# laizesheng1/Monte-Carlo-Path-Tracer

Measured on AMD Instinct MI355X. Metric: Mray/s (primary+secondary), cornell-box 1024spp, higher is better.
Workload: dtype f32; 1 GPU; S-cornell (synthetic cornell-box.obj stand-in, 39612 tris) 800x800, depth=8, 1024 spp per step, MIS integrator, reference-faithful shadow rays; spp_per_rank=1024, n_tris=39612, wide_bvh=8-wide, 4220 nodes, depth 9, scene_device_bytes=21940128, parallelism=sample-range shard x1 + RCCL all-reduce of the 800x800x4 fp32 film

## Files before the change

### monte-carlo-path-tracer_amd/csrc/device_scene.h

```cpp
#pragma once
#include <stdint.h>
#include <hip/hip_runtime.h>

#ifndef MCPT_Q_MARGIN
#define MCPT_Q_MARGIN (1.0 / 1024.0)
#endif
#ifndef MCPT_LEAF_MAX
#define MCPT_LEAF_MAX 2
#endif
#ifndef MCPT_STACK_DEPTH
#define MCPT_STACK_DEPTH 64
#endif
#ifndef MCPT_BLOCK
#define MCPT_BLOCK 256
#endif
#ifndef MCPT_TOP_NODES
#define MCPT_TOP_NODES 256
#endif
#define MCPT_NODE_SENTINEL ((int)0x80000000)
#define HIT_CLASS_SHIFT 28
#define HIT_TRI_MASK 0x0fffffff
#define HIT_CLASS_DIFFUSE 0u
#define HIT_CLASS_PHONG 1u
#define HIT_CLASS_MIRROR 2u
// ... 29 lines not shown
#define MCPT_N8_WORD(slot) ((slot) >> 1)
#define MCPT_N8_LO_SHIFT(slot) (8 * ((slot) & 1))
#define MCPT_N8_HI_SHIFT(slot) (16 + 8 * ((slot) & 1))
#define MCPT_N8_EMPTY_WORD 0x0000ffffu
#define MCPT_TRI_SHADE_F4 8
struct DevScene {
    const float4* nodes;
    const float4* nodes8;
    const float4* tri_isect;
    const float4* tri_shade;
    const double* tri_pos64;
    const int32_t* tri_face;
    const DevMaterial* mats;
    const DevLight* lights;
    const double* light_pos64;
    const float4* texels;
    DevCamera cam;
    double centre[3];
    int32_t n_tris, n_lights, n_nodes, n_mats, n_nodes8;
};

struct RenderParams {
    uint32_t spp;
    uint32_t first_sample;
    uint32_t samples_per_item;
    uint32_t chunks;
    uint32_t tiles_x, tiles_y;
    uint32_t tile_mod, tile_rem;
    uint32_t n_owned;
    uint32_t max_depth;
    uint32_t flags;
    uint32_t integrator;
    uint32_t seed_lo, seed_hi;
    uint32_t atomic_accum;
// ... 16 lines not shown
```

### monte-carlo-path-tracer_amd/csrc/mcpt_api.cpp

```cpp
#include "../../include/mcpt.h"
#include "kernels.h"
#include "scene_build.h"
#include "bvh_gpu.h"
#include "wavefront.h"
#include "denoise.h"
#include "adaptive.h"
#include "refit.h"

#include <chrono>
#include <cmath>
#include <cstdlib>
#include <cstdio>
#include <cstring>
#include <memory>
#include <string>
#include <vector>

namespace {

thread_local std::string g_err;

template <class H, auto Free> struct Owned {
    H h = nullptr;
    Owned() = default;
// ... 16 lines not shown
    void release() { if (p) { (void)hipFree(p); if (tally) *tally -= bytes; } p = nullptr; bytes = 0; }
    hipError_t alloc(size_t n, uint64_t* count = nullptr) {
        release();
        const hipError_t e = hipMalloc(&p, n ? n : 16);
        if (e == hipSuccess) { bytes = n; tally = count; if (tally) *tally += n; } else p = nullptr;
        return e;
    }
};

}

struct mcpt_ctx {
    int device = 0;
    mcpt_opts opts{};
    DevScene dev{};
    DevBuf nodes, nodes8, tri_isect, tri_shade, tri_pos64, tri_face, mats, lights, light_pos64, texels, accum_own, counters;
    float4* accum = nullptr;
    Stream own_stream; hipStream_t stream = nullptr;
    static constexpr uint32_t TIMED = 16;
    Event ev0[TIMED], ev1[TIMED];
    uint32_t timed_head = 0, timed_tail = 0;
    double last_kernel_ms = 0.0, total_kernel_ms = 0.0;
    uint64_t launches = 0;
    mcpt_scene_info info{};
    int width = 0, height = 0;
    bool use_wavefront = true;
    struct WfLane {
        PathPool pool{};
        CompactBufs compact{};
        std::vector<DevBuf> pool_bufs;
        DevBuf ctl_buf, ovf_buf;
// ... 169 lines not shown
                HIP_TRY(hipStreamCreateWithFlags(L.stream.out(), hipStreamNonBlocking));
                const size_t ovf_bytes = size_t(c->trace_grid) * wf_trace_block_threads() * wf_trace_overflow_bytes_per_lane(c->wide_depth);
                if (ovf_bytes > (size_t(512) << 20)) return fail(MCPT_ERR_BVH_DEPTH, "wide BVH of depth " + std::to_string(c->wide_depth) + " needs a traversal-stack overflow area of " + std::to_string(ovf_bytes >> 20) + " MB per sub-pipeline: build the tree with the host builder (no MCPT_FLAG_GPU_BVH_BUILD)");
                HIP_TRY(L.ovf_buf.alloc(ovf_bytes));
            }
        }
    }
    HIP_TRY(hipDeviceSynchronize());
    c->accum = static_cast<float4*>(c->accum_own.p);
    DevScene& d = c->dev;
    d.nodes = static_cast<const float4*>(c->nodes.p); d.nodes8 = static_cast<const float4*>(c->nodes8.p);
    d.tri_isect = static_cast<const float4*>(c->tri_isect.p);
    d.tri_shade = static_cast<const float4*>(c->tri_shade.p); d.tri_pos64 = static_cast<const double*>(c->tri_pos64.p);
    d.tri_face = static_cast<const int32_t*>(c->tri_face.p); d.mats = static_cast<const DevMaterial*>(c->mats.p);
    d.lights = static_cast<const DevLight*>(c->lights.p); d.light_pos64 = static_cast<const double*>(c->light_pos64.p); d.texels = static_cast<const float4*>(c->texels.p);
    return MCPT_OK;
}

static void fill_wide_info(mcpt_scene_info& in, const HostScene& hs) {
    in.wide_width = 8; in.wide_nodes = uint32_t(hs.nodes8.size() / 5);
    in.wide_depth = hs.bvh8_depth;
    in.traversal_bytes = (hs.nodes8.size() + hs.tri_isect.size()) * sizeof(f4h);
    for (int a = 0; a < 3; a++) in.centre[a] = hs.centre[a];
    uint64_t h = 1469598103934665603ull;
    auto mix = [&](const void* p, size_t bytes) { const uint32_t* w = static_cast<const uint32_t*>(p); for (size_t i = 0; i < bytes / 4; i++) { h ^= w[i]; h *= 1099511628211ull; } };
    mix(hs.nodes8.data(), hs.nodes8.size() * sizeof(f4h)); mix(hs.tri_face.data(), hs.tri_face.size() * 4);
    in.wide_tree_hash = h;
}


// ... 100 lines not shown
        if ((st = check_device(o.device)) != MCPT_OK) return st;
    }

    if ((hs.nodes8.size() * sizeof(f4h) >= (1ull << 32) || hs.tri_isect.size() * sizeof(f4h) >= (1ull << 32)))
        return fail(MCPT_ERR_UNSUPPORTED, "scene too large for the 8-wide traversal kernel (more than 89 M triangles)");
    std::unique_ptr<mcpt_ctx, void (*)(mcpt_ctx*)> guard(new mcpt_ctx(), destroy_ctx);
    mcpt_ctx* c = guard.get();
    c->device = o.device; c->opts = o; c->width = scene->camera.width; c->height = scene->camera.height;
    c->wide_depth = hs.bvh8_depth; c->binary_ok = hs.binary_ok; c->use_wavefront = use_wavefront;
    HIP_TRY(hipSetDevice(c->device));
    auto t0 = std::chrono::steady_clock::now();
    uint64_t* tally = &c->info.device_bytes;
    HIP_TRY(upload(c->nodes, hs.nodes, tally)); HIP_TRY(upload(c->nodes8, hs.nodes8, tally)); HIP_TRY(upload(c->tri_isect, hs.tri_isect, tally));
    HIP_TRY(upload(c->tri_shade, hs.tri_shade, tally)); HIP_TRY(upload(c->tri_pos64, hs.tri_pos64, tally)); HIP_TRY(upload(c->tri_face, hs.tri_face, tally));
    HIP_TRY(upload(c->mats, hs.mats, tally)); HIP_TRY(upload(c->lights, hs.lights, tally)); HIP_TRY(upload(c->light_pos64, hs.light_pos64, tally));
    HIP_TRY(upload(c->texels, hs.texels, tally));
    DevScene& d = c->dev;
    d.n_nodes8 = int32_t(hs.nodes8.size() / 5);
    d.cam = hs.cam;
    for (int a = 0; a < 3; a++) d.centre[a] = hs.centre[a];
    d.n_tris = int32_t(hs.tri_face.size()); d.n_lights = int32_t(hs.lights.size()); d.n_nodes = int32_t(hs.nodes.size() / 4); d.n_mats = int32_t(hs.mats.size());
    mcpt_scene_info& in = c->info;
    in.n_tris = uint32_t(d.n_tris); in.n_lights = uint32_t(d.n_lights); in.n_nodes = uint32_t(d.n_nodes);
    in.bvh_depth = hs.bvh_depth; in.max_leaf = hs.max_leaf; in.width = uint32_t(c->width); in.height = uint32_t(c->height);
    in.bvh_build_ms = hs.bvh_build_ms;
    fill_wide_info(in, hs);
    if ((st = finish_ctx(c)) != MCPT_OK) return st;
    if ((o.flags & MCPT_FLAG_DYNAMIC) && (st = rf_setup(c, hs, scene)) != MCPT_OK) return st;
    in.upload_ms = std::chrono::duration<double, std::milli>(std::chrono::steady_clock::now() - t0).count();
    *out_ctx = guard.release();
    return MCPT_OK;
}

mcpt_status mcpt_clone_to_device(mcpt_ctx* src, int32_t device, mcpt_ctx** out_ctx) {
    if (!src || !out_ctx) return fail(MCPT_ERR_INVALID_ARG, "mcpt_clone_to_device: null argument");
    *out_ctx = nullptr;
    mcpt_status st = check_device(device); if (st != MCPT_OK) return st;
    st = use(src); if (st != MCPT_OK) return st;
    HIP_TRY(hipStreamSynchronize(src->stream));
    std::unique_ptr<mcpt_ctx, void (*)(mcpt_ctx*)> guard(new mcpt_ctx(), destroy_ctx);
    mcpt_ctx* c = guard.get();
    c->device = device; c->opts = src->opts; c->opts.device = device; c->width = src->width; c->height = src->height;
    c->wide_depth = src->wide_depth; c->binary_ok = src->binary_ok; c->use_wavefront = src->use_wavefront;
    c->dev = src->dev; c->info = src->info; c->info.bvh_build_ms = 0.0; c->info.device_bytes = 0;
    HIP_TRY(hipSetDevice(device));
    auto t0 = std::chrono::steady_clock::now();
    DevBuf* from[10] = {&src->nodes, &src->nodes8, &src->tri_isect, &src->tri_shade, &src->tri_pos64, &src->tri_face, &src->mats, &src->lights, &src->light_pos64, &src->texels};
    DevBuf* to[10] = {&c->nodes, &c->nodes8, &c->tri_isect, &c->tri_shade, &c->tri_pos64, &c->tri_face, &c->mats, &c->lights, &c->light_pos64, &c->texels};
    for (int i = 0; i < 10; i++) {
        HIP_TRY(to[i]->alloc(from[i]->bytes, &c->info.device_bytes));
        if (from[i]->bytes) HIP_TRY(hipMemcpyPeer(to[i]->p, device, from[i]->p, src->device, from[i]->bytes));
    }
    if ((st = finish_ctx(c)) != MCPT_OK) return st;
    if (src->dynamic && (st = rf_clone(c, src)) != MCPT_OK) return st;
    c->info.upload_ms = std::chrono::duration<double, std::milli>(std::chrono::steady_clock::now() - t0).count();
    *out_ctx = guard.release();
    return MCPT_OK;
}

mcpt_status mcpt_destroy(mcpt_ctx* ctx) {
    if (!ctx) return MCPT_OK;
    (void)hipSetDevice(ctx->device);
    (void)hipDeviceSynchronize();
    destroy_ctx(ctx);
// ... 625 lines not shown
    if (ctx->rf_timed) { HIP_TRY(hipEventSynchronize(ctx->rf_ev1)); float ms = 0.f; HIP_TRY(hipEventElapsedTime(&ms, ctx->rf_ev0, ctx->rf_ev1)); ctx->rf_last_ms = ms; ctx->rf_timed = false; }
    const size_t vd = size_t(n_vertex) * 3, nd = size_t(ctx->rf_n_normal) * 3;
    std::memcpy(ctx->rf_stage, vertex, vd * sizeof(double));
    if (normal) std::memcpy(ctx->rf_stage + vd, normal, nd * sizeof(double));
    hipStream_t s = ctx->stream;
    HIP_TRY(hipEventRecord(ctx->rf_ev0, s));
    HIP_TRY(hipMemcpyAsync(ctx->rf_vtx.p, ctx->rf_stage, vd * sizeof(double), hipMemcpyHostToDevice, s));
    if (normal) HIP_TRY(hipMemcpyAsync(ctx->rf_nrm.p, ctx->rf_stage + vd, nd * sizeof(double), hipMemcpyHostToDevice, s));
    HIP_TRY(hipEventRecord(ctx->rf_stage_ev, s)); ctx->rf_stage_pending = true;
    const double* d_nrm = normal ? static_cast<const double*>(ctx->rf_nrm.p) : nullptr;
    const int32_t* idx = static_cast<const int32_t*>(ctx->rf_idx.p);
    float* tri_box = static_cast<float*>(ctx->rf_tri_box.p);
    const DevScene& d = ctx->dev;
    HIP_TRY(launch_rf_triangles(static_cast<const double*>(ctx->rf_vtx.p), d_nrm, idx, RfCentre{d.centre[0], d.centre[1], d.centre[2]}, static_cast<float4*>(ctx->tri_isect.p),
                                static_cast<float4*>(ctx->tri_shade.p), static_cast<double*>(ctx->tri_pos64.p), tri_box, uint32_t(d.n_tris), s));
    HIP_TRY(launch_rf_lights(static_cast<DevLight*>(ctx->lights.p), static_cast<double*>(ctx->light_pos64.p), d.tri_isect, d.tri_pos64, d_nrm, idx, uint32_t(d.n_lights), s));
    for (size_t k = 0; k + 1 < ctx->rf_bin_level.size(); k++)
        HIP_TRY(launch_rf_binary_level(static_cast<float4*>(ctx->nodes.p), static_cast<const uint32_t*>(ctx->rf_bin_order.p), ctx->rf_bin_level[k], ctx->rf_bin_level[k + 1], tri_box, s));
    for (size_t k = ctx->rf_wide_level.size() - 1; k-- > 0;)
        HIP_TRY(launch_rf_wide_level(static_cast<float4*>(ctx->nodes8.p), ctx->rf_wide_level[k], ctx->rf_wide_level[k + 1], tri_box, static_cast<float*>(ctx->rf_node_box.p), s));
    HIP_TRY(launch_rf_wide_area(d.nodes8, uint32_t(d.n_nodes8), static_cast<double*>(ctx->rf_area.p), s));
    HIP_TRY(hipEventRecord(ctx->rf_ev1, s)); ctx->rf_timed = true;
    ctx->rf_updates++;
    rf_forget_derived(ctx);
    return MCPT_OK;
}

mcpt_status mcpt_get_update_info(mcpt_ctx* ctx, mcpt_update_info* out) {
    mcpt_status st = use(ctx); if (st != MCPT_OK) return st;
    if (!out) return fail(MCPT_ERR_INVALID_ARG, "null output");
    HIP_TRY(hipStreamSynchronize(ctx->stream));
// ... 231 lines not shown
```

### monte-carlo-path-tracer_amd/csrc/refit.h

```cpp
#pragma once
#include <hip/hip_runtime.h>
#include "device_scene.h"

#define RF_BLOCK 256

struct RfCentre { double x, y, z; };

hipError_t launch_rf_triangles(const double* vertex, const double* normal, const int32_t* idx6, RfCentre centre, float4* tri_isect, float4* tri_shade,
                               double* tri_pos64, float* tri_box, uint32_t n_tris, hipStream_t stream);
hipError_t launch_rf_lights(DevLight* lights, double* light_pos64, const float4* tri_isect, const double* tri_pos64, const double* normal,
                            const int32_t* idx6, uint32_t n_lights, hipStream_t stream);
hipError_t launch_rf_binary_level(float4* nodes, const uint32_t* order, uint32_t begin, uint32_t end, const float* tri_box, hipStream_t stream);
hipError_t launch_rf_wide_level(float4* nodes8, uint32_t begin, uint32_t end, const float* tri_box, float* node_box, hipStream_t stream);
hipError_t launch_rf_wide_area(const float4* nodes8, uint32_t n_nodes8, double* partial, hipStream_t stream);
inline uint32_t rf_area_blocks(uint32_t n_nodes8) { return (n_nodes8 + RF_BLOCK - 1) / RF_BLOCK; }
```

### monte-carlo-path-tracer_amd/csrc/refit.hip

```cpp
#include "refit.h"

#pragma clang fp contract(off)

namespace {

__device__ __forceinline__ float rf_down(double v) { float f = (float)v; if ((double)f > v) f = nextafterf(f, -INFINITY); return f; }
__device__ __forceinline__ float rf_up(double v) { float f = (float)v; if ((double)f < v) f = nextafterf(f, INFINITY); return f; }

struct RfBox { float lo[3], hi[3]; };
__device__ __forceinline__ RfBox rf_load_box(const float* __restrict__ boxes, size_t i) {
    const float2* p = reinterpret_cast<const float2*>(boxes + 6 * i);
    const float2 a = p[0], b = p[1], c = p[2];
    return RfBox{{a.x, a.y, b.x}, {b.y, c.x, c.y}};
}
__device__ __forceinline__ void rf_store_box(float* __restrict__ boxes, size_t i, const RfBox& b) {
    float2* p = reinterpret_cast<float2*>(boxes + 6 * i);
    p[0] = make_float2(b.lo[0], b.lo[1]); p[1] = make_float2(b.lo[2], b.hi[0]); p[2] = make_float2(b.hi[1], b.hi[2]);
}
__device__ __forceinline__ void rf_grow(RfBox& a, const RfBox& b) {
    for (int x = 0; x < 3; x++) { a.lo[x] = fminf(a.lo[x], b.lo[x]); a.hi[x] = fmaxf(a.hi[x], b.hi[x]); }
}
__device__ __forceinline__ RfBox rf_leaf_box(const float* __restrict__ tri_box, uint32_t first, uint32_t cnt) {
    RfBox b = rf_load_box(tri_box, first);
    for (uint32_t t = 1; t < cnt; t++) rf_grow(b, rf_load_box(tri_box, (size_t)first + t));
// ... 30 lines not shown
    }
    double* P = tri_pos64 + 9 * (size_t)i;
    for (int a = 0; a < 3; a++) { P[a] = v0[a]; P[3 + a] = v1[a]; P[6 + a] = v2[a]; }
    {
        const double ax = v1[0] - v0[0], ay = v1[1] - v0[1], az = v1[2] - v0[2], bx = v2[0] - v0[0], by = v2[1] - v0[1], bz = v2[2] - v0[2];
        const double nx = ay * bz - by * az, ny = az * bx - bz * ax, nz = ax * by - bx * ay;
        const double d = nx * v0[0] + ny * v0[1] + nz * v0[2];
        double2* pl = reinterpret_cast<double2*>(S + 4);
        pl[0] = make_double2(nx, ny); pl[1] = make_double2(nz, d);
    }
    RfBox b;
    for (int a = 0; a < 3; a++) { b.lo[a] = rf_down(fmin(v0[a], fmin(v1[a], v2[a]))); b.hi[a] = rf_up(fmax(v0[a], fmax(v1[a], v2[a]))); }
    rf_store_box(tri_box, i, b);
}

__global__ void __launch_bounds__(RF_BLOCK) rf_lights_kernel(DevLight* __restrict__ lights, double* __restrict__ light_pos64, const float4* __restrict__ tri_isect,
                                                             const double* __restrict__ tri_pos64, const double* __restrict__ normal, const int32_t* __restrict__ idx6,
                                                             uint32_t n_lights) {
    const uint32_t i = blockIdx.x * RF_BLOCK + threadIdx.x;
    if (i >= n_lights) return;
    float4* R = reinterpret_cast<float4*>(lights + i);
    float4 r0 = R[0], r1 = R[1], r2 = R[2], r3 = R[3];
    const uint32_t tri = (uint32_t)__float_as_int(r0.x);
    const float4 e1 = tri_isect[3 * (size_t)tri + 1], e2 = tri_isect[3 * (size_t)tri + 2];
    const float cx = e1.y * e2.z - e2.y * e1.z, cy = e1.z * e2.x - e2.z * e1.x, cz = e1.x * e2.y - e2.x * e1.y;
    r0.y = 0.5f * (float)sqrt((double)((cx * cx + cy * cy) + cz * cz));
    if (normal) {
        const int32_t* ix = idx6 + 6 * (size_t)tri + 3;
        const double* n0 = normal + 3 * (size_t)ix[0]; const double* n1 = normal + 3 * (size_t)ix[1]; const double* n2 = normal + 3 * (size_t)ix[2];
        r1.y = (float)n0[0]; r1.z = (float)n0[1]; r1.w = (float)n0[2];
        r2.x = (float)n1[0]; r2.y = (float)n1[1]; r2.z = (float)n1[2];
        r2.w = (float)n2[0]; r3.x = (float)n2[1]; r3.y = (float)n2[2];
    }
    R[0] = r0; R[1] = r1; R[2] = r2; R[3] = r3;
    for (int a = 0; a < 9; a++) light_pos64[9 * (size_t)i + a] = tri_pos64[9 * (size_t)tri + a];
}

__global__ void __launch_bounds__(RF_BLOCK) rf_binary_kernel(float4* __restrict__ nodes, const uint32_t* __restrict__ order, uint32_t begin, uint32_t end,
                                                             const float* __restrict__ tri_box) {
    const uint32_t k = begin + blockIdx.x * RF_BLOCK + threadIdx.x;
    if (k >= end) return;
    float4* N = nodes + 4 * (size_t)order[k];
    const float4 a0 = N[0], a1 = N[1], az = N[2], links = N[3];
    RfBox b[2] = {{{a0.x, a0.z, az.x}, {a0.y, a0.w, az.y}}, {{a1.x, a1.z, az.z}, {a1.y, a1.w, az.w}}};
#pragma unroll
    for (int c = 0; c < 2; c++) {
        const int code = __float_as_int(c == 0 ? links.x : links.y);
        if (code >= 0) {
            const float4* C = nodes + 4 * (size_t)code;
            const float4 c0 = C[0], c1 = C[1], cz = C[2];
// ... 99 lines not shown
    __syncthreads();
    if (threadIdx.x == 0) { double t = 0.0; for (int w = 0; w < RF_BLOCK / 64; w++) t += s_sum[w]; partial[blockIdx.x] = t; }
}

inline dim3 rf_grid(uint32_t n) { return dim3((n + RF_BLOCK - 1) / RF_BLOCK); }

}

hipError_t launch_rf_triangles(const double* vertex, const double* normal, const int32_t* idx6, RfCentre centre, float4* tri_isect, float4* tri_shade,
                               double* tri_pos64, float* tri_box, uint32_t n_tris, hipStream_t stream) {
    if (n_tris == 0) return hipSuccess;
    hipLaunchKernelGGL(rf_triangles_kernel, rf_grid(n_tris), dim3(RF_BLOCK), 0, stream, vertex, normal, idx6, centre, tri_isect, tri_shade, tri_pos64, tri_box, n_tris);
    return hipGetLastError();
}

hipError_t launch_rf_lights(DevLight* lights, double* light_pos64, const float4* tri_isect, const double* tri_pos64, const double* normal,
                            const int32_t* idx6, uint32_t n_lights, hipStream_t stream) {
    if (n_lights == 0) return hipSuccess;
    hipLaunchKernelGGL(rf_lights_kernel, rf_grid(n_lights), dim3(RF_BLOCK), 0, stream, lights, light_pos64, tri_isect, tri_pos64, normal, idx6, n_lights);
    return hipGetLastError();
}

hipError_t launch_rf_binary_level(float4* nodes, const uint32_t* order, uint32_t begin, uint32_t end, const float* tri_box, hipStream_t stream) {
    if (end <= begin) return hipSuccess;
    hipLaunchKernelGGL(rf_binary_kernel, rf_grid(end - begin), dim3(RF_BLOCK), 0, stream, nodes, order, begin, end, tri_box);
    return hipGetLastError();
}

hipError_t launch_rf_wide_level(float4* nodes8, uint32_t begin, uint32_t end, const float* tri_box, float* node_box, hipStream_t stream) {
    if (end <= begin) return hipSuccess;
    hipLaunchKernelGGL(rf_wide_kernel, rf_grid(end - begin), dim3(RF_BLOCK), 0, stream, nodes8, begin, end, tri_box, node_box);
    return hipGetLastError();
}

// ... 6 lines not shown
```

### monte-carlo-path-tracer_amd/csrc/scene_build.cpp

```cpp
#include "scene_build.h"

#include <algorithm>
#include <atomic>
#include <chrono>
#include <future>
#include <cmath>
#include <cstdio>
#include <cstdlib>
#include <cstring>
#include <limits>
#include <system_error>
#include <thread>

static constexpr double kMaxCoord = MCPT_MAX_COORD;

namespace {

struct BTri { double lo[3], hi[3], c[3]; };
struct Box {
    double lo[3], hi[3];
    Box() { for (int a = 0; a < 3; a++) { lo[a] = std::numeric_limits<double>::max(); hi[a] = std::numeric_limits<double>::lowest(); } }
    void grow(const double* l, const double* h) { for (int a = 0; a < 3; a++) { lo[a] = std::min(lo[a], l[a]); hi[a] = std::max(hi[a], h[a]); } }
    void grow(const Box& b) { grow(b.lo, b.hi); }
    void grow_pt(const double* p) { for (int a = 0; a < 3; a++) { lo[a] = std::min(lo[a], p[a]); hi[a] = std::max(hi[a], p[a]); } }
// ... 658 lines not shown
        S[1] = {float(n1[0]), float(n1[1]), float(n1[2]), float(t0_[1])};
        S[2] = {float(n2[0]), float(n2[1]), float(n2[2]), float(t1_[0])};
        S[3] = {float(t1_[1]), float(t2_[0]), float(t2_[1]), as_float(c[3])};
        for (int a = 0; a < 3; a++) { out.tri_pos64[9 * size_t(i) + a] = v0[a]; out.tri_pos64[9 * size_t(i) + 3 + a] = v1[a]; out.tri_pos64[9 * size_t(i) + 6 + a] = v2[a]; }
        {
            const double ax = v1[0] - v0[0], ay = v1[1] - v0[1], az = v1[2] - v0[2], bx = v2[0] - v0[0], by = v2[1] - v0[1], bz = v2[2] - v0[2];
            const double nx = ay * bz - by * az, ny = az * bx - bz * ax, nz = ax * by - bx * ay;
            const double pl[4] = {nx, ny, nz, nx * v0[0] + ny * v0[1] + nz * v0[2]};
            std::memcpy(&S[4], pl, sizeof pl);
        }
        out.tri_face[i] = f;
        if (out.keep_dynamic) for (int k = 0; k < 3; k++) { out.dyn_idx[6 * size_t(i) + k] = c[4 * k]; out.dyn_idx[6 * size_t(i) + 3 + k] = c[4 * k + 1]; }
    }
    });

    out.lights.clear(); out.light_pos64.clear();
    for (uint32_t f = 0; f < nf; f++) {
        const int32_t* c = d->face + 12 * size_t(f);
        const mcpt_material& m = d->materials[c[3]];
        if (!(len3(m.radiance) > 0.01)) continue;
        DevLight L; std::memset(&L, 0, sizeof L);
        L.tri = pos_of_face[f];
        const f4h e1 = out.tri_isect[3 * size_t(L.tri) + 1], e2 = out.tri_isect[3 * size_t(L.tri) + 2];
        const float cx = e1.y * e2.z - e2.y * e1.z, cy = e1.z * e2.x - e2.z * e1.x, cz = e1.x * e2.y - e2.x * e1.y;
        L.area = 0.5f * std::sqrt((cx * cx + cy * cy) + cz * cz);
        for (int a = 0; a < 3; a++) {
            L.radiance[a] = float(m.radiance[a]);
            L.n0[a] = float(d->normal[3 * size_t(c[1]) + a]); L.n1[a] = float(d->normal[3 * size_t(c[5]) + a]); L.n2[a] = float(d->normal[3 * size_t(c[9]) + a]);
        }
        out.lights.push_back(L);
        out.light_pos64.insert(out.light_pos64.end(), out.tri_pos64.begin() + 9 * size_t(L.tri), out.tri_pos64.begin() + 9 * size_t(L.tri) + 9);
    }
    if (out.lights.empty()) { err = "scene has no emissive triangle (|radiance| > 0.01); the reference indexes lights[-1] here"; return MCPT_ERR_NO_LIGHTS; }

    camera_constants(d->camera, ctr, out.cam);
    return MCPT_OK;
}
```

### monte-carlo-path-tracer_amd/csrc/scene_build.h

```cpp
#pragma once
#include <cstdint>
#include <functional>
#include <string>
#include <vector>
#include "../../include/mcpt.h"
#include "device_scene.h"

struct f4h { float x, y, z, w; };

struct HostScene {
    std::vector<f4h> nodes;
    std::vector<f4h> nodes8;
    std::vector<f4h> tri_isect;
    std::vector<f4h> tri_shade;
    std::vector<double> tri_pos64;
    std::vector<int32_t> tri_face;
    std::vector<DevMaterial> mats;
    std::vector<DevLight> lights;
    std::vector<double> light_pos64;
    std::vector<f4h> texels;
    DevCamera cam;
    double centre[3] = {0.0, 0.0, 0.0};
    uint32_t bvh_depth = 0, max_leaf = 0, bvh8_depth = 0;
    std::vector<int> subtree_begin;
    bool reference_tie_order = false;
    bool allow_deep_binary = false;
    bool binary_ok = true;
    double bvh_build_ms = 0.0;
    bool keep_dynamic = false;
    std::vector<int32_t> dyn_idx;
};

using BvhBuildFn = std::function<bool(const float* boxes, uint32_t n, std::vector<f4h>& nodes, std::vector<int>& order, uint32_t& depth,
                                      uint32_t& max_leaf, std::string& err)>;
// ... 15 lines not shown
```

### monte-carlo-path-tracer_amd/csrc/wavefront.h

```cpp
#pragma once
#include <hip/hip_runtime.h>
#include <stdint.h>
#include "device_scene.h"

#ifndef WF_SHADE_BLOCK
#define WF_SHADE_BLOCK 256
#endif
#define SLOT_DEAD  0u
#define SLOT_ALIVE 1u
#define SLOT_DRAIN 2u

struct PathPool {
    float4* ray_o;
    float4* ray_d;
    float4* hit;
    float4* sq_o;
    float4* sq_d;
    float4* nee;
    float4* L;
    float4* beta;
    float4* sum;
    uint4* ids;
    uint32_t* shadow_queue;
    uint32_t* shadow_count;
    uint32_t* live_cnt;
// ... 55 lines not shown
```

### monte-carlo-path-tracer_amd/csrc/wavefront.hip

```cpp
#include "pt_device.h"
#include "wavefront.h"

typedef float wf_v4f __attribute__((ext_vector_type(4)));
typedef unsigned int wf_v4u __attribute__((ext_vector_type(4)));
typedef double wf_v2d __attribute__((ext_vector_type(2)));
__device__ __forceinline__ float4 ld_s(const float4* p) { const wf_v4f v = __builtin_nontemporal_load(reinterpret_cast<const wf_v4f*>(p)); return make_float4(v.x, v.y, v.z, v.w); }
__device__ __forceinline__ void st_s(float4* p, float4 v) { wf_v4f t; t.x = v.x; t.y = v.y; t.z = v.z; t.w = v.w; __builtin_nontemporal_store(t, reinterpret_cast<wf_v4f*>(p)); }
__device__ __forceinline__ uint4 ld_s(const uint4* p) { const wf_v4u v = __builtin_nontemporal_load(reinterpret_cast<const wf_v4u*>(p)); return make_uint4(v.x, v.y, v.z, v.w); }
__device__ __forceinline__ void st_s(uint4* p, uint4 v) { wf_v4u t; t.x = v.x; t.y = v.y; t.z = v.z; t.w = v.w; __builtin_nontemporal_store(t, reinterpret_cast<wf_v4u*>(p)); }
__device__ __forceinline__ double4 ld_s(const double4* p) {
    const wf_v2d a = __builtin_nontemporal_load(reinterpret_cast<const wf_v2d*>(p)), b = __builtin_nontemporal_load(reinterpret_cast<const wf_v2d*>(p) + 1);
    return make_double4(a.x, a.y, b.x, b.y);
}
__device__ __forceinline__ void st_s(double4* p, double4 v) {
    wf_v2d a, b; a.x = v.x; a.y = v.y; b.x = v.z; b.y = v.w;
    __builtin_nontemporal_store(a, reinterpret_cast<wf_v2d*>(p)); __builtin_nontemporal_store(b, reinterpret_cast<wf_v2d*>(p) + 1);
}
typedef unsigned int wf_v2u __attribute__((ext_vector_type(2)));
__device__ __forceinline__ uint2 ld_s(const uint2* p) { const wf_v2u v = __builtin_nontemporal_load(reinterpret_cast<const wf_v2u*>(p)); return make_uint2(v.x, v.y); }
__device__ __forceinline__ void st_s(uint2* p, uint2 v) { wf_v2u t; t.x = v.x; t.y = v.y; __builtin_nontemporal_store(t, reinterpret_cast<wf_v2u*>(p)); }
__device__ __forceinline__ uint32_t ld_s(const uint32_t* p) { return __builtin_nontemporal_load(p); }
__device__ __forceinline__ void st_s(uint32_t* p, uint32_t v) { __builtin_nontemporal_store(v, p); }
__device__ __forceinline__ f3 xyz(const float4 v) { return mk3(v.x, v.y, v.z); }
__device__ __forceinline__ float4 mk4(f3 v, float w) { return make_float4(v.x, v.y, v.z, w); }
// ... 39 lines not shown
    { const uint32_t p_act = ctl->pad[WF_CTL_P_ACTIVE]; if ((it != 0u && ctl->any_active[(it - 1u) & 3u] == 0u) || (p_act != 0u && base >= p_act)) return; }
    __shared__ uint32_t s_wave_cnt[WF_SHADE_BLOCK / 64], s_shadow_cnt[WF_SHADE_BLOCK / 64], s_live_cnt[WF_SHADE_BLOCK / 64];
    __shared__ uint32_t s_base, s_sel, s_scan, s_priv_base, s_priv_take, s_priv_next, s_priv_end;
    __shared__ float4 s_beta[WF_SHADE_BLOCK], s_hit[WF_SHADE_BLOCK], s_L[WF_SHADE_BLOCK], s_rd[WF_SHADE_BLOCK], s_nee[WF_SHADE_BLOCK], s_ro[WF_SHADE_BLOCK];
    __shared__ uint2 s_ids[WF_SHADE_BLOCK];
    uint2* const id_ps = reinterpret_cast<uint2*>(pool.ids);
    uint2* const id_ne = id_ps + pool.P;
#define OUT_RAY_O 2u
#define OUT_SHADOW 4u
#define OUT_IDS 8u
    __shared__ uint32_t s_perm[WF_SHADE_BLOCK];
    __shared__ uint32_t s_kcnt[K_COUNT * (WF_SHADE_BLOCK / 64)];
    __shared__ float4 s_mats[WF_LDS_MATS * 4];
    __shared__ float4 s_lights[WF_LDS_LIGHTS * 4];
    __shared__ double s_light_pos[WF_LDS_LIGHTS * 9];
    const bool mats_lds = sc.n_mats <= WF_LDS_MATS, lights_lds = sc.n_lights <= WF_LDS_LIGHTS;

    {
        const float4 bt0 = ld_s(&pool.beta[base + tid]), h0 = ld_s(&pool.hit[base + tid]);
        const uint2 id0 = ld_s(&id_ps[base + tid]);
        const float4 L0 = ld_s(&pool.L[base + tid]), rd0 = ld_s(&pool.ray_d[base + tid]), nee0 = ld_s(&pool.nee[base + tid]), ro0 = ld_s(&pool.ray_o[base + tid]);
        uint2 priv = make_uint2(0u, 0u);
        if (tid == 0 && p.priv_items) {
            if (it == 0) { priv.x = 0u; priv.y = p.priv_items; }
            else priv = pool.block_items[blockIdx.x];
        }
        if (mats_lds) for (uint32_t i = tid; i < (uint32_t)sc.n_mats * 4; i += WF_SHADE_BLOCK) s_mats[i] = reinterpret_cast<const float4*>(sc.mats)[i];
        if (lights_lds) {
            for (uint32_t i = tid; i < (uint32_t)sc.n_lights * 4; i += WF_SHADE_BLOCK) s_lights[i] = reinterpret_cast<const float4*>(sc.lights)[i];
            for (uint32_t i = tid; i < (uint32_t)sc.n_lights * 9; i += WF_SHADE_BLOCK) s_light_pos[i] = sc.light_pos64[i];
        }
        s_L[tid] = L0; s_rd[tid] = rd0; s_nee[tid] = nee0; s_ro[tid] = ro0;
        if (tid == 0) { s_priv_next = priv.x; s_priv_end = priv.y; }
        s_beta[tid] = bt0; s_hit[tid] = h0; s_ids[tid] = id0;
        const uint32_t st0 = __float_as_uint(bt0.w);
        const int bounce0 = (int)(st0 >> 8), tri0 = __float_as_int(h0.x);
        uint32_t key = K_END;
        if ((st0 & 3u) == SLOT_ALIVE && tri0 >= 0) {
            bool ends = p.max_depth != 0 && (uint32_t)bounce0 >= p.max_depth;
            if (bounce0 - 1 > 3) {
                const float q = fminf(max3(xyz(bt0)), 0.95f);
                const Rng4 r = rng_block(id0.x, id0.y, 2u + 2u * (uint32_t)(bounce0 - 1), p.seed_lo, p.seed_hi);
                ends = ends || r.v[2] > q;
            }
            key = ends ? K_EMIT : K_DIFF + ((uint32_t)tri0 >> HIT_CLASS_SHIFT);
        }
        uint32_t my_rank = 0;
#pragma unroll
        for (uint32_t k = 0; k < K_COUNT; k++) {
            const uint64_t m = __ballot(key == k);
            if (key == k) my_rank = lane_rank(m);
            if (lane == k) s_kcnt[k * (WF_SHADE_BLOCK / 64) + wv] = (uint32_t)__popcll(m);
        }
        __syncthreads();
        const uint32_t my_cell = key * (WF_SHADE_BLOCK / 64) + wv;
        static_assert(K_COUNT * (WF_SHADE_BLOCK / 64) <= 32, "the scan covers two DPP rows");
        const uint32_t cell_cnt = lane < K_COUNT * (WF_SHADE_BLOCK / 64) ? s_kcnt[lane] : 0u;
        int inc = (int)cell_cnt;
        inc += __builtin_amdgcn_update_dpp(0, inc, 0x111, 0xf, 0xf, true);
        inc += __builtin_amdgcn_update_dpp(0, inc, 0x112, 0xf, 0xf, true);
// ... 7 lines not shown
    const uint32_t pk = s_perm[tid];
    const uint32_t key = pk >> 16, src = pk & 0xffffu, slot = base + src;
    SH_TICK(0)

#define WF_PHASE() asm volatile("" ::: "memory")
    const uint32_t st = __float_as_uint(s_beta[src].w);
    uint32_t state = st & 3u;
    bool prev_mirror = (st & 4u) != 0;
    int bounce = (int)(st >> 8);
    float4 sm = make_float4(0.f, 0.f, 0.f, 0.f); bool sm_loaded = false;
    const float nl = (float)sc.n_lights;
    const bool correct_t2 = (p.flags & MCPT_FLAG_CORRECT_SHADOW_T2) != 0;

    bool terminated = false, emit_extend = false, emit_shadow = false, sum_dirty = false, id_dirty = false;
    bool c_prim = false, c_cont = false, c_self_t = false, c_self_h = false, c_shaded = false;
    uint32_t c_texel = 0;
    uint32_t out_flags = 0;

    if (state != SLOT_DEAD && (st & 8u) != 0) {
        const float4 n4 = s_nee[src];
        if (__float_as_uint(n4.w) == 0u) { float4 L4 = s_L[src]; L4.x += n4.x; L4.y += n4.y; L4.z += n4.z; s_L[src] = L4; }
    }
    if (key != K_END) do {
        int tri;
        double4 plane64;
        f3 kd_early = mk3(0.f, 0.f, 0.f);
        {
            const float4 h = s_hit[src];
            tri = __float_as_int(h.x) & HIT_TRI_MASK;
            plane64 = *reinterpret_cast<const double4*>(sc.tri_shade + MCPT_TRI_SHADE_F4 * (size_t)tri + 4);
// ... 65 lines not shown
        }
        int sh_skip = -1;
        if (ls.pdf != 0.f) {
            c_self_t = true; c_self_h = ls.self_hit;
            if (correct_t2 || !ls.self_hit) {
                f3 fx; float bpdf;
                bsdf_eval(bsdf, ls.wo, fx, bpdf);
                const float cos_theta = fabsf(dot(bsdf.w, ls.wo));
                const float weight = power_heuristic(ls.pdf * rcp(nl), bpdf);
                const f3 nee = weight * xyz(s_beta[src]) * ls.rad * fx * (cos_theta * rcp(ls.pdf) * nl);
                s_hit[src] = mk4(ls.wo, ls.t2); s_nee[src] = mk4(nee, 0.f); out_flags |= OUT_SHADOW;
                sh_skip = ls.tri; emit_shadow = true;
            }
        }
        s_ro[src] = mk4(p32, __int_as_float(sh_skip)); out_flags |= OUT_RAY_O;
        Scatter s;
        {
            const uint2 id = s_ids[src];
            const Rng4 rb = rng_block(id.x, id.y, 2u + 2u * (uint32_t)bounce, p.seed_lo, p.seed_hi);
            s = bsdf_sample(bsdf, xi_lobe, rb.v[0], rb.v[1]);
        }
        if (s.pdf == 0.f) {
            state = SLOT_DRAIN;
            break;
        }
        {
            const float sc_ = fabsf(dot(bsdf.w, s.wo)) * rcp(s.pdf);
            float4 b4 = s_beta[src];
            b4.x *= s.f.x * sc_; b4.y *= s.f.y * sc_; b4.z *= s.f.z * sc_;
            s_beta[src] = b4;
            float4 L4 = s_L[src]; L4.w = s.pdf; s_L[src] = L4;
        }
        prev_mirror = s.mirror;
        s_rd[src] = mk4(s.wo, 0.f); bounce++;
        emit_extend = true; c_cont = true;
    } while (0);
    else if (state != SLOT_DEAD) terminated = true;
    WF_PHASE();
    SH_TICK(3)
    uint4 id;
    { const uint2 ps = s_ids[src]; id.x = ps.x; id.y = ps.y; id.z = id.w = 0u; }
    const bool multi = p.samples_per_item != 1u && p.probe_n == 0u;
    if (multi && (terminated || state == SLOT_DEAD)) { const uint2 ne = ld_s(&id_ne[slot]); id.z = ne.x; id.w = ne.y; }

    if (p.samples_per_item != 1u && (terminated || (state == SLOT_DEAD && id.z == id.w))) { sm = ld_s(&pool.sum[slot]); sm_loaded = true; }
    if (terminated) {
        const f3 c = wf_scrub_nan(xyz(s_L[src]));
        sm.x += c.x; sm.y += c.y; sm.z += c.z; sm.w += 1.f; sum_dirty = true;
        state = SLOT_DEAD;
    }
// ... 69 lines not shown
    }
    if (state == SLOT_DEAD && id.z < id.w) {
        id.y = id.z++; id_dirty = true;
        d3 eye64; f3 no, nd;
        if (p.probe_n) {
            eye64 = mkd(p.probe_o[3 * id.x], p.probe_o[3 * id.x + 1], p.probe_o[3 * id.x + 2]); no = to_f3(eye64);
            nd = mk3((float)p.probe_d[3 * id.x], (float)p.probe_d[3 * id.x + 1], (float)p.probe_d[3 * id.x + 2]);
        } else {
            const Rng4 r = rng_block(id.x, id.y, 0u, p.seed_lo, p.seed_hi);
            const int py = (int)wf_fastdiv(id.x, p.div_width_m, p.div_width_s), px = (int)(id.x - (uint32_t)py * (uint32_t)sc.cam.width);
            cast_ray(sc.cam, px, py, r.v[0], r.v[1], eye64, no, nd);
        }
        s_ro[src] = mk4(no, __int_as_float(-1)); out_flags |= OUT_RAY_O;
        s_rd[src] = mk4(nd, 0.f);
        s_beta[src] = make_float4(1.f, 1.f, 1.f, 0.f); s_L[src] = make_float4(0.f, 0.f, 0.f, 0.f);
        bounce = 0; prev_mirror = false;
        state = SLOT_ALIVE; emit_extend = true; c_prim = true;
    }

    SH_TICK(4)
    {
        float4 b4 = s_beta[src];
        b4.w = __uint_as_float(state | (prev_mirror ? 4u : 0u) | (emit_shadow ? 8u : 0u) | ((uint32_t)bounce << 8));
        s_beta[src] = b4;
        if (sum_dirty && sm_loaded) st_s(&pool.sum[slot], sm);
        if (id_dirty) { s_ids[src] = make_uint2(id.x, id.y); out_flags |= OUT_IDS; if (multi) st_s(&id_ne[slot], make_uint2(id.z, id.w)); }
        float4 r4 = s_rd[src];
        r4.w = __uint_as_float(out_flags | (emit_extend ? 1u : 0u));
        s_rd[src] = r4;
    }

    const uint32_t cur = it & 3;
    const uint64_t ms = __ballot(emit_shadow);
    const uint32_t n_live = (uint32_t)__popcll(__ballot(state != SLOT_DEAD));
    if (lane == 0) { s_shadow_cnt[wv] = (uint32_t)__popcll(ms); s_live_cnt[wv] = n_live; }
    __syncthreads();
    if (tid == 0) {
        uint32_t tot = 0, live = 0;
// ... 7 lines not shown
        st_s(&pool.shadow_queue[q], slot); st_s(&pool.sq_o[q], s_ro[src]); st_s(&pool.sq_d[q], s_hit[src]);
    }
    {
        const uint32_t own = base + tid;
        const float4 rdo = s_rd[tid];
        const uint32_t fl = __float_as_uint(rdo.w);
        st_s(&pool.beta[own], s_beta[tid]); st_s(&pool.L[own], s_L[tid]); st_s(&pool.ray_d[own], rdo);
        if (fl & OUT_RAY_O) st_s(&pool.ray_o[own], s_ro[tid]);
        if (fl & OUT_SHADOW) st_s(&pool.nee[own], s_nee[tid]);
        if (fl & OUT_IDS) st_s(&id_ps[own], s_ids[tid]);
    }
    SH_TICK(5)
    const uint64_t ma = __ballot(state != SLOT_DEAD);
    const uint64_t m_term = __ballot(terminated), m_prim = __ballot(c_prim), m_cont = __ballot(c_cont);
    const uint64_t m_st = __ballot(c_self_t), m_sh = __ballot(c_self_h), m_shaded = __ballot(c_shaded);
    unsigned long long texels = 0;
    if (COUNT) { texels = c_texel; for (int off = 32; off > 0; off >>= 1) texels += __shfl_xor(texels, off, 64); }
    if (lane == 0) {
        DevCounters* g = gcnt + (blockIdx.x & (WF_COUNTER_REPLICAS - 1));
        if (ma) ctl->any_active[cur] = 1u;
#ifndef WF_SCHED_STATS
        if (m_term) atomicAdd(&g->paths, (unsigned long long)__popcll(m_term));
#endif
        if (m_prim) atomicAdd(&g->rays_primary, (unsigned long long)__popcll(m_prim));
        if (m_cont) atomicAdd(&g->rays_continuation, (unsigned long long)__popcll(m_cont));
        if (ms) atomicAdd(&g->rays_shadow, (unsigned long long)__popcll(ms));
#ifndef WF_SCHED_STATS
        if (m_st) atomicAdd(&g->self_shadow_tests, (unsigned long long)__popcll(m_st));
        if (m_sh) atomicAdd(&g->self_shadow_hits, (unsigned long long)__popcll(m_sh));
#endif
#ifndef WF_SCHED_STATS
        if (COUNT) { if (m_shaded) atomicAdd(&g->shaded_hits, (unsigned long long)__popcll(m_shaded)); if (texels) atomicAdd(&g->texel_fetches, texels); }
#endif
#ifdef WF_SHADE_STATS
        SH_TICK(6)
        atomicAdd(&g->debug[0], sh_t[0]); atomicAdd(&g->debug[1], sh_t[1]); atomicAdd(&g->debug[2], sh_t[2]); atomicAdd(&g->debug[3], sh_t[3]);
        atomicAdd(&g->box_tests, sh_t[4]); atomicAdd(&g->tri_tests, sh_t[5]); atomicAdd(&g->stack_spills, sh_t[6]); atomicAdd(&g->texel_fetches, 1ull);
#endif
    }
}
#undef SH_TICK

#ifndef WF_TRACE_BLOCK
#define WF_TRACE_BLOCK 1024
#endif
#ifndef WF_CHUNK_BATCH
#define WF_CHUNK_BATCH 4
// ... 455 lines not shown
```

Before: 10570 Mray/s.

## Cull final path segments whose continuation ray cannot reach any emitter

Moves the Russian-roulette and max-depth termination decision from the next shade pass into the scatter step and stores it as a SLOT_ENDS flag. When a path's next segment is known to be its last and every emitter triangle is in the light list, the continuation ray is tested against all light triangles held in LDS. If it misses them all, the path is drained without tracing that ray, since the segment could only add emission. This saves BVH traversals for final bounces at the cost of a per-light triangle loop and a light_isect buffer. Correctness depends on the emitter-completeness check and on occlusion being irrelevant when the ray misses every light.

```diff
diff --git a/monte-carlo-path-tracer_amd/csrc/device_scene.h b/monte-carlo-path-tracer_amd/csrc/device_scene.h
--- a/monte-carlo-path-tracer_amd/csrc/device_scene.h
+++ b/monte-carlo-path-tracer_amd/csrc/device_scene.h
@@ -67,10 +67,13 @@
     const DevMaterial* mats;
     const DevLight* lights;
     const double* light_pos64;
+    const float4* light_isect;
     const float4* texels;
     DevCamera cam;
     double centre[3];
     int32_t n_tris, n_lights, n_nodes, n_mats, n_nodes8;
+    int32_t emitters_listed;
+    int32_t cull_last_segments;
 };
 
 struct RenderParams {
diff --git a/monte-carlo-path-tracer_amd/csrc/mcpt_api.cpp b/monte-carlo-path-tracer_amd/csrc/mcpt_api.cpp
--- a/monte-carlo-path-tracer_amd/csrc/mcpt_api.cpp
+++ b/monte-carlo-path-tracer_amd/csrc/mcpt_api.cpp
@@ -54,7 +54,7 @@
     int device = 0;
     mcpt_opts opts{};
     DevScene dev{};
-    DevBuf nodes, nodes8, tri_isect, tri_shade, tri_pos64, tri_face, mats, lights, light_pos64, texels, accum_own, counters;
+    DevBuf nodes, nodes8, tri_isect, tri_shade, tri_pos64, tri_face, mats, lights, light_pos64, light_isect, texels, accum_own, counters;
     float4* accum = nullptr;
     Stream own_stream; hipStream_t stream = nullptr;
     static constexpr uint32_t TIMED = 16;
@@ -254,6 +254,8 @@
     d.tri_shade = static_cast<const float4*>(c->tri_shade.p); d.tri_pos64 = static_cast<const double*>(c->tri_pos64.p);
     d.tri_face = static_cast<const int32_t*>(c->tri_face.p); d.mats = static_cast<const DevMaterial*>(c->mats.p);
     d.lights = static_cast<const DevLight*>(c->lights.p); d.light_pos64 = static_cast<const double*>(c->light_pos64.p); d.texels = static_cast<const float4*>(c->texels.p);
+    d.light_isect = static_cast<const float4*>(c->light_isect.p);
+    d.cull_last_segments = (d.emitters_listed && d.n_lights <= WF_LDS_LIGHTS && env_u32("MCPT_NO_LAST_SEGMENT_CULL", 0) == 0) ? 1 : 0;
     return MCPT_OK;
 }
 
@@ -384,12 +386,14 @@
     HIP_TRY(upload(c->nodes, hs.nodes, tally)); HIP_TRY(upload(c->nodes8, hs.nodes8, tally)); HIP_TRY(upload(c->tri_isect, hs.tri_isect, tally));
     HIP_TRY(upload(c->tri_shade, hs.tri_shade, tally)); HIP_TRY(upload(c->tri_pos64, hs.tri_pos64, tally)); HIP_TRY(upload(c->tri_face, hs.tri_face, tally));
     HIP_TRY(upload(c->mats, hs.mats, tally)); HIP_TRY(upload(c->lights, hs.lights, tally)); HIP_TRY(upload(c->light_pos64, hs.light_pos64, tally));
+    HIP_TRY(upload(c->light_isect, hs.light_isect, tally));
     HIP_TRY(upload(c->texels, hs.texels, tally));
     DevScene& d = c->dev;
     d.n_nodes8 = int32_t(hs.nodes8.size() / 5);
     d.cam = hs.cam;
     for (int a = 0; a < 3; a++) d.centre[a] = hs.centre[a];
     d.n_tris = int32_t(hs.tri_face.size()); d.n_lights = int32_t(hs.lights.size()); d.n_nodes = int32_t(hs.nodes.size() / 4); d.n_mats = int32_t(hs.mats.size());
+    d.emitters_listed = hs.emitters_listed ? 1 : 0;
     mcpt_scene_info& in = c->info;
     in.n_tris = uint32_t(d.n_tris); in.n_lights = uint32_t(d.n_lights); in.n_nodes = uint32_t(d.n_nodes);
     in.bvh_depth = hs.bvh_depth; in.max_leaf = hs.max_leaf; in.width = uint32_t(c->width); in.height = uint32_t(c->height);
@@ -415,9 +419,9 @@
     c->dev = src->dev; c->info = src->info; c->info.bvh_build_ms = 0.0; c->info.device_bytes = 0;
     HIP_TRY(hipSetDevice(device));
     auto t0 = std::chrono::steady_clock::now();
-    DevBuf* from[10] = {&src->nodes, &src->nodes8, &src->tri_isect, &src->tri_shade, &src->tri_pos64, &src->tri_face, &src->mats, &src->lights, &src->light_pos64, &src->texels};
-    DevBuf* to[10] = {&c->nodes, &c->nodes8, &c->tri_isect, &c->tri_shade, &c->tri_pos64, &c->tri_face, &c->mats, &c->lights, &c->light_pos64, &c->texels};
-    for (int i = 0; i < 10; i++) {
+    DevBuf* from[11] = {&src->nodes, &src->nodes8, &src->tri_isect, &src->tri_shade, &src->tri_pos64, &src->tri_face, &src->mats, &src->lights, &src->light_pos64, &src->light_isect, &src->texels};
+    DevBuf* to[11] = {&c->nodes, &c->nodes8, &c->tri_isect, &c->tri_shade, &c->tri_pos64, &c->tri_face, &c->mats, &c->lights, &c->light_pos64, &c->light_isect, &c->texels};
+    for (int i = 0; i < 11; i++) {
         HIP_TRY(to[i]->alloc(from[i]->bytes, &c->info.device_bytes));
         if (from[i]->bytes) HIP_TRY(hipMemcpyPeer(to[i]->p, device, from[i]->p, src->device, from[i]->bytes));
     }
@@ -1073,7 +1077,7 @@
     const DevScene& d = ctx->dev;
     HIP_TRY(launch_rf_triangles(static_cast<const double*>(ctx->rf_vtx.p), d_nrm, idx, RfCentre{d.centre[0], d.centre[1], d.centre[2]}, static_cast<float4*>(ctx->tri_isect.p),
                                 static_cast<float4*>(ctx->tri_shade.p), static_cast<double*>(ctx->tri_pos64.p), tri_box, uint32_t(d.n_tris), s));
-    HIP_TRY(launch_rf_lights(static_cast<DevLight*>(ctx->lights.p), static_cast<double*>(ctx->light_pos64.p), d.tri_isect, d.tri_pos64, d_nrm, idx, uint32_t(d.n_lights), s));
+    HIP_TRY(launch_rf_lights(static_cast<DevLight*>(ctx->lights.p), static_cast<double*>(ctx->light_pos64.p), static_cast<float4*>(ctx->light_isect.p), d.tri_isect, d.tri_pos64, d_nrm, idx, uint32_t(d.n_lights), s));
     for (size_t k = 0; k + 1 < ctx->rf_bin_level.size(); k++)
         HIP_TRY(launch_rf_binary_level(static_cast<float4*>(ctx->nodes.p), static_cast<const uint32_t*>(ctx->rf_bin_order.p), ctx->rf_bin_level[k], ctx->rf_bin_level[k + 1], tri_box, s));
     for (size_t k = ctx->rf_wide_level.size() - 1; k-- > 0;)
diff --git a/monte-carlo-path-tracer_amd/csrc/refit.h b/monte-carlo-path-tracer_amd/csrc/refit.h
--- a/monte-carlo-path-tracer_amd/csrc/refit.h
+++ b/monte-carlo-path-tracer_amd/csrc/refit.h
@@ -8,7 +8,7 @@
 
 hipError_t launch_rf_triangles(const double* vertex, const double* normal, const int32_t* idx6, RfCentre centre, float4* tri_isect, float4* tri_shade,
                                double* tri_pos64, float* tri_box, uint32_t n_tris, hipStream_t stream);
-hipError_t launch_rf_lights(DevLight* lights, double* light_pos64, const float4* tri_isect, const double* tri_pos64, const double* normal,
+hipError_t launch_rf_lights(DevLight* lights, double* light_pos64, float4* light_isect, const float4* tri_isect, const double* tri_pos64, const double* normal,
                             const int32_t* idx6, uint32_t n_lights, hipStream_t stream);
 hipError_t launch_rf_binary_level(float4* nodes, const uint32_t* order, uint32_t begin, uint32_t end, const float* tri_box, hipStream_t stream);
 hipError_t launch_rf_wide_level(float4* nodes8, uint32_t begin, uint32_t end, const float* tri_box, float* node_box, hipStream_t stream);
diff --git a/monte-carlo-path-tracer_amd/csrc/refit.hip b/monte-carlo-path-tracer_amd/csrc/refit.hip
--- a/monte-carlo-path-tracer_amd/csrc/refit.hip
+++ b/monte-carlo-path-tracer_amd/csrc/refit.hip
@@ -68,7 +68,7 @@
     rf_store_box(tri_box, i, b);
 }
 
-__global__ void __launch_bounds__(RF_BLOCK) rf_lights_kernel(DevLight* __restrict__ lights, double* __restrict__ light_pos64, const float4* __restrict__ tri_isect,
+__global__ void __launch_bounds__(RF_BLOCK) rf_lights_kernel(DevLight* __restrict__ lights, double* __restrict__ light_pos64, float4* __restrict__ light_isect, const float4* __restrict__ tri_isect,
                                                              const double* __restrict__ tri_pos64, const double* __restrict__ normal, const int32_t* __restrict__ idx6,
                                                              uint32_t n_lights) {
     const uint32_t i = blockIdx.x * RF_BLOCK + threadIdx.x;
@@ -88,6 +88,7 @@
     }
     R[0] = r0; R[1] = r1; R[2] = r2; R[3] = r3;
     for (int a = 0; a < 9; a++) light_pos64[9 * (size_t)i + a] = tri_pos64[9 * (size_t)tri + a];
+    light_isect[3 * (size_t)i] = tri_isect[3 * (size_t)tri]; light_isect[3 * (size_t)i + 1] = e1; light_isect[3 * (size_t)i + 2] = e2;
 }
 
 __global__ void __launch_bounds__(RF_BLOCK) rf_binary_kernel(float4* __restrict__ nodes, const uint32_t* __restrict__ order, uint32_t begin, uint32_t end,
@@ -217,10 +218,10 @@
     return hipGetLastError();
 }
 
-hipError_t launch_rf_lights(DevLight* lights, double* light_pos64, const float4* tri_isect, const double* tri_pos64, const double* normal,
+hipError_t launch_rf_lights(DevLight* lights, double* light_pos64, float4* light_isect, const float4* tri_isect, const double* tri_pos64, const double* normal,
                             const int32_t* idx6, uint32_t n_lights, hipStream_t stream) {
     if (n_lights == 0) return hipSuccess;
-    hipLaunchKernelGGL(rf_lights_kernel, rf_grid(n_lights), dim3(RF_BLOCK), 0, stream, lights, light_pos64, tri_isect, tri_pos64, normal, idx6, n_lights);
+    hipLaunchKernelGGL(rf_lights_kernel, rf_grid(n_lights), dim3(RF_BLOCK), 0, stream, lights, light_pos64, light_isect, tri_isect, tri_pos64, normal, idx6, n_lights);
     return hipGetLastError();
 }
 
diff --git a/monte-carlo-path-tracer_amd/csrc/scene_build.cpp b/monte-carlo-path-tracer_amd/csrc/scene_build.cpp
--- a/monte-carlo-path-tracer_amd/csrc/scene_build.cpp
+++ b/monte-carlo-path-tracer_amd/csrc/scene_build.cpp
@@ -696,11 +696,11 @@
     }
     });
 
-    out.lights.clear(); out.light_pos64.clear();
+    out.lights.clear(); out.light_pos64.clear(); out.light_isect.clear(); out.emitters_listed = true;
     for (uint32_t f = 0; f < nf; f++) {
         const int32_t* c = d->face + 12 * size_t(f);
         const mcpt_material& m = d->materials[c[3]];
-        if (!(len3(m.radiance) > 0.01)) continue;
+        if (!(len3(m.radiance) > 0.01)) { if (out.mats[size_t(c[3])].flags & MAT_EMISSIVE) out.emitters_listed = false; continue; }
         DevLight L; std::memset(&L, 0, sizeof L);
         L.tri = pos_of_face[f];
         const f4h e1 = out.tri_isect[3 * size_t(L.tri) + 1], e2 = out.tri_isect[3 * size_t(L.tri) + 2];
@@ -712,6 +712,7 @@
         }
         out.lights.push_back(L);
         out.light_pos64.insert(out.light_pos64.end(), out.tri_pos64.begin() + 9 * size_t(L.tri), out.tri_pos64.begin() + 9 * size_t(L.tri) + 9);
+        out.light_isect.insert(out.light_isect.end(), out.tri_isect.begin() + 3 * size_t(L.tri), out.tri_isect.begin() + 3 * size_t(L.tri) + 3);
     }
     if (out.lights.empty()) { err = "scene has no emissive triangle (|radiance| > 0.01); the reference indexes lights[-1] here"; return MCPT_ERR_NO_LIGHTS; }
 
diff --git a/monte-carlo-path-tracer_amd/csrc/scene_build.h b/monte-carlo-path-tracer_amd/csrc/scene_build.h
--- a/monte-carlo-path-tracer_amd/csrc/scene_build.h
+++ b/monte-carlo-path-tracer_amd/csrc/scene_build.h
@@ -18,6 +18,8 @@
     std::vector<DevMaterial> mats;
     std::vector<DevLight> lights;
     std::vector<double> light_pos64;
+    std::vector<f4h> light_isect;
+    bool emitters_listed = true;
     std::vector<f4h> texels;
     DevCamera cam;
     double centre[3] = {0.0, 0.0, 0.0};
diff --git a/monte-carlo-path-tracer_amd/csrc/wavefront.h b/monte-carlo-path-tracer_amd/csrc/wavefront.h
--- a/monte-carlo-path-tracer_amd/csrc/wavefront.h
+++ b/monte-carlo-path-tracer_amd/csrc/wavefront.h
@@ -9,6 +9,7 @@
 #define SLOT_DEAD  0u
 #define SLOT_ALIVE 1u
 #define SLOT_DRAIN 2u
+#define SLOT_ENDS 16u
 
 struct PathPool {
     float4* ray_o;
diff --git a/monte-carlo-path-tracer_amd/csrc/wavefront.hip b/monte-carlo-path-tracer_amd/csrc/wavefront.hip
--- a/monte-carlo-path-tracer_amd/csrc/wavefront.hip
+++ b/monte-carlo-path-tracer_amd/csrc/wavefront.hip
@@ -77,6 +77,7 @@
     __shared__ float4 s_mats[WF_LDS_MATS * 4];
     __shared__ float4 s_lights[WF_LDS_LIGHTS * 4];
     __shared__ double s_light_pos[WF_LDS_LIGHTS * 9];
+    __shared__ float4 s_light_isect[WF_LDS_LIGHTS * 3];
     const bool mats_lds = sc.n_mats <= WF_LDS_MATS, lights_lds = sc.n_lights <= WF_LDS_LIGHTS;
 
     {
@@ -92,6 +93,7 @@
         if (lights_lds) {
             for (uint32_t i = tid; i < (uint32_t)sc.n_lights * 4; i += WF_SHADE_BLOCK) s_lights[i] = reinterpret_cast<const float4*>(sc.lights)[i];
             for (uint32_t i = tid; i < (uint32_t)sc.n_lights * 9; i += WF_SHADE_BLOCK) s_light_pos[i] = sc.light_pos64[i];
+            for (uint32_t i = tid; i < (uint32_t)sc.n_lights * 3; i += WF_SHADE_BLOCK) s_light_isect[i] = sc.light_isect[i];
         }
         s_L[tid] = L0; s_rd[tid] = rd0; s_nee[tid] = nee0; s_ro[tid] = ro0;
         if (tid == 0) { s_priv_next = priv.x; s_priv_end = priv.y; }
@@ -100,13 +102,7 @@
         const int bounce0 = (int)(st0 >> 8), tri0 = __float_as_int(h0.x);
         uint32_t key = K_END;
         if ((st0 & 3u) == SLOT_ALIVE && tri0 >= 0) {
-            bool ends = p.max_depth != 0 && (uint32_t)bounce0 >= p.max_depth;
-            if (bounce0 - 1 > 3) {
-                const float q = fminf(max3(xyz(bt0)), 0.95f);
-                const Rng4 r = rng_block(id0.x, id0.y, 2u + 2u * (uint32_t)(bounce0 - 1), p.seed_lo, p.seed_hi);
-                ends = ends || r.v[2] > q;
-            }
-            key = ends ? K_EMIT : K_DIFF + ((uint32_t)tri0 >> HIT_CLASS_SHIFT);
+            key = (st0 & SLOT_ENDS) ? K_EMIT : K_DIFF + ((uint32_t)tri0 >> HIT_CLASS_SHIFT);
         }
         uint32_t my_rank = 0;
 #pragma unroll
@@ -144,6 +140,7 @@
 
     bool terminated = false, emit_extend = false, emit_shadow = false, sum_dirty = false, id_dirty = false;
     bool c_prim = false, c_cont = false, c_self_t = false, c_self_h = false, c_shaded = false;
+    bool ends = false, c_last = false, c_culled = false;
     uint32_t c_texel = 0;
     uint32_t out_flags = 0;
 
@@ -239,11 +236,12 @@
             }
         }
         s_ro[src] = mk4(p32, __int_as_float(sh_skip)); out_flags |= OUT_RAY_O;
-        Scatter s;
+        Scatter s; float xi_rr;
         {
             const uint2 id = s_ids[src];
             const Rng4 rb = rng_block(id.x, id.y, 2u + 2u * (uint32_t)bounce, p.seed_lo, p.seed_hi);
             s = bsdf_sample(bsdf, xi_lobe, rb.v[0], rb.v[1]);
+            xi_rr = rb.v[2];
         }
         if (s.pdf == 0.f) {
             state = SLOT_DRAIN;
@@ -255,10 +253,29 @@
             b4.x *= s.f.x * sc_; b4.y *= s.f.y * sc_; b4.z *= s.f.z * sc_;
             s_beta[src] = b4;
             float4 L4 = s_L[src]; L4.w = s.pdf; s_L[src] = L4;
+            bounce++;
+            ends = p.max_depth != 0 && (uint32_t)bounce >= p.max_depth;
+            if (bounce - 1 > 3) ends = ends || xi_rr > fminf(max3(xyz(b4)), 0.95f);
         }
         prev_mirror = s.mirror;
-        s_rd[src] = mk4(s.wo, 0.f); bounce++;
-        emit_extend = true; c_cont = true;
+        s_rd[src] = mk4(s.wo, 0.f);
+        c_cont = true; c_last = ends;
+        if (ends && sc.cull_last_segments) {
+            WF_PHASE();
+            const f3 ro = xyz(s_ro[src]), rd = xyz(s_rd[src]);
+            bool faces_light = false;
+#pragma unroll 1
+            for (int li = 0; li < sc.n_lights; li++) {
+                const TriTest r = tri_test(s_light_isect[3 * li], s_light_isect[3 * li + 1], s_light_isect[3 * li + 2], ro, rd);
+                faces_light = faces_light || tri_accept_closest(r, 1e-4f, 3.0e38f);
+            }
+            if (!faces_light) {
+                c_culled = true; ends = false;
+                state = SLOT_DRAIN;
+                break;
+            }
+        }
+        emit_extend = true;
     } while (0);
     else if (state != SLOT_DEAD) terminated = true;
     WF_PHASE();
@@ -358,14 +375,14 @@
         s_ro[src] = mk4(no, __int_as_float(-1)); out_flags |= OUT_RAY_O;
         s_rd[src] = mk4(nd, 0.f);
         s_beta[src] = make_float4(1.f, 1.f, 1.f, 0.f); s_L[src] = make_float4(0.f, 0.f, 0.f, 0.f);
-        bounce = 0; prev_mirror = false;
+        bounce = 0; prev_mirror = false; ends = false;
         state = SLOT_ALIVE; emit_extend = true; c_prim = true;
     }
 
     SH_TICK(4)
     {
         float4 b4 = s_beta[src];
-        b4.w = __uint_as_float(state | (prev_mirror ? 4u : 0u) | (emit_shadow ? 8u : 0u) | ((uint32_t)bounce << 8));
+        b4.w = __uint_as_float(state | (prev_mirror ? 4u : 0u) | (emit_shadow ? 8u : 0u) | (ends ? SLOT_ENDS : 0u) | ((uint32_t)bounce << 8));
         s_beta[src] = b4;
         if (sum_dirty && sm_loaded) st_s(&pool.sum[slot], sm);
         if (id_dirty) { s_ids[src] = make_uint2(id.x, id.y); out_flags |= OUT_IDS; if (multi) st_s(&id_ne[slot], make_uint2(id.z, id.w)); }
@@ -403,6 +420,7 @@
     const uint64_t ma = __ballot(state != SLOT_DEAD);
     const uint64_t m_term = __ballot(terminated), m_prim = __ballot(c_prim), m_cont = __ballot(c_cont);
     const uint64_t m_st = __ballot(c_self_t), m_sh = __ballot(c_self_h), m_shaded = __ballot(c_shaded);
+    const uint64_t m_last = COUNT ? __ballot(c_last) : 0ull, m_culled = COUNT ? __ballot(c_culled) : 0ull;
     unsigned long long texels = 0;
     if (COUNT) { texels = c_texel; for (int off = 32; off > 0; off >>= 1) texels += __shfl_xor(texels, off, 64); }
     if (lane == 0) {
@@ -420,6 +438,12 @@
 #endif
 #ifndef WF_SCHED_STATS
         if (COUNT) { if (m_shaded) atomicAdd(&g->shaded_hits, (unsigned long long)__popcll(m_shaded)); if (texels) atomicAdd(&g->texel_fetches, texels); }
+#endif
+#if !defined(WF_SCHED_STATS) && !defined(WF_SHADE_STATS)
+        if (COUNT) {
+            if (m_last) atomicAdd(&g->debug[2], (unsigned long long)__popcll(m_last));
+            if (m_culled) atomicAdd(&g->debug[3], (unsigned long long)__popcll(m_culled));
+        }
 #endif
 #ifdef WF_SHADE_STATS
         SH_TICK(6)
```

Measured after the change: 10400 Mray/s. -1.6%, worse.
